# gengshan-y/ppr-diffphys

Hardware: AMD Instinct MI355X
Metric: env-steps/sec (fwd+adjoint), Laikago 12-DoF, batch=4096, 1/2/4/8 MI355X (higher is better)
Workload: dtype f32; 1 GPU; laikago, mixed mi-trot/mi-spin mocap targets, 4096 envs in total (4096 on rank 0) x 100 sim steps (4 frames), dt=5e-4, fwd+adjoint, batch split only (no collective); global_batch=4096, envs_per_gpu=4096, sim_steps=100, segment_lanes=16, nan_grads=0

## Files before the change

### ppr-diffphys_amd/csrc/pd_args.h

```cpp
#pragma once
#include "pd_device.h"
#include "pd_trajloss.h"

#define PD_BWAVES 4
#define PD_BLOCK (2 * PD_BWAVES * 64)
#define PD_FK_BLOCK (PD_BWAVES * 64)
#define PD_BLOCK3 (3 * PD_BWAVES * 64)

#define PD_HITLOG 32

enum { PD_K_ROLLOUT_FWD = 0, PD_K_ROLLOUT_BWD = 1, PD_K_FK_FWD = 2, PD_K_FK_BWD = 3,
       PD_K_REDUCE_FK = 4, PD_K_SEEDS_FK = 5 };
#define PD_REDUCE_BLOCK 1024

constexpr bool pd_split(int jt) { return jt == PD_JT_REVOLUTE; }
constexpr bool pd_parented(int jt) { return jt == PD_JT_REVOLUTE || jt == PD_JT_COMPOUND; }
enum { PD_KV_FWD_SPLIT = 0, PD_KV_FWD_UNSPLIT, PD_KV_BWD_2ROLE, PD_KV_BWD3_2ROLE, PD_KV_FK,
       PD_KV_FWD_QUAD, PD_KV_BWD_QUAD };
struct PdLaunchCfg {
  int kernel;
  int roles;
  int groups;
  int nblocks, threads;
  size_t lds;
};
inline int pd_groups_per_wg(int n_groups, int cu_count) {
  int g = cu_count > 0 ? (n_groups + cu_count - 1) / cu_count : PD_BWAVES;
  return g < 1 ? 1 : (g > PD_BWAVES ? PD_BWAVES : g);
}
inline int pd_kernel_variant(int kind, int jt, int n_groups, int cu_count) {
  if (kind == PD_K_ROLLOUT_FWD) return (jt != PD_JT_COMPOUND || n_groups <= PD_BWAVES * cu_count) ? PD_KV_FWD_SPLIT : PD_KV_FWD_UNSPLIT;
  if (kind == PD_K_ROLLOUT_BWD) {
    return pd_split(jt) ? PD_KV_BWD_2ROLE : PD_KV_BWD3_2ROLE;
  }
  return PD_KV_FK;
}
#define PD_CULLW_MIN_CAP 48
inline int pd_fwd_cull_cap(int nb, int segw, int list_cap, int env_lds_floats, int rec, int w6) {
  const int spec_off = ((4 + rec + 2 * w6) * nb + w6 + 3) & ~3;
  return env_lds_floats - (spec_off + 8 * nb + 4 + list_cap + 8 * segw + 6 * segw + 8 * segw);
}
inline int pd_variant_roles(int kv) {
  return (kv == PD_KV_FWD_UNSPLIT || kv == PD_KV_FK) ? 1 : 2;
}

#define PD_TRAJ_FLOATS 20

struct RolloutArgs {
  int bs, nsteps, nframes;
  float dt;
  const float *q_init, *qd_init, *torques, *res_f, *refs, *target_ke, *target_kd, *inv_mass, *inertia, *inv_inertia;
  const float *state0;
  float *g_state0;
  const int *frame_of_step;
  float *ws;
  float *wp_pos, *wp_vel, *grf, *jaf;
  const float *adj_pos, *adj_vel;
  float *g_q_init, *g_qd_init, *g_torques, *g_res_f, *g_refs, *g_ke, *g_kd, *g_inv_mass, *g_inertia, *g_inv_inertia;
  int *hitlog;
  const float *loss_target;
  const unsigned char *loss_outseq;
  float loss_rot_ratio;
  float *loss_seed_pos, *loss_seed_gt, *loss_table;
  unsigned long long *dbg;
};


struct FkArgs {
  int n;
  const float *joint_q, *joint_qd;
  float *body_q, *body_qd;
  const float *adj_body_q, *adj_body_qd;
  float *g_joint_q, *g_joint_qd;
  int perm_bs;
};
struct ReduceFkArgs { FkArgs fk; TrajReduceArgs red; int in_lds; };
struct SeedsFkArgs { FkArgs fk; TrajSeedsArgs seeds; };

// ... 14 lines not shown
```

### ppr-diffphys_amd/csrc/pd_host.hip

```cpp
#include <algorithm>
#include <cmath>
#include <cstdio>
#include <cstring>
#include <string>
#include <vector>

#include "../../include/ppr_diffphys.h"
#include "pd_args.h"

static thread_local std::string g_err;
static int fail(const std::string &msg) { g_err = msg; return 1; }
__attribute__((visibility("hidden"))) int pd_set_error(const char *msg) { return fail(msg); }
static int hip_fail(hipError_t e, const char *what) { return fail(std::string(what) + ": " + hipGetErrorString(e)); }

struct pd_model {
  int nb = 0, nq = 0, nqd = 0, nc = 0, nmat = 0;
  std::vector<int> jtype, jparent, qstart, qdstart, cbody, cmat;
  std::vector<float> X_p, X_c, axis, com, lim_lo, lim_hi, lim_ke, lim_kd, cpoint, cdist, materials;
  float gravity[3] = {0, 0, 0}, attach_ke = 0, attach_kd = 0;
  int segw = 0, jt = 0;
  std::vector<int> contact_order;
  struct Quad { void *blob; PdDevModel dev; size_t lds_tables; int jt; };
  Quad *quad = nullptr;
  int policy = 0;
// ... 270 lines not shown
  void *blob = nullptr;
  hipError_t e = hipMalloc(&blob, b.buf.size());
  if (e != hipSuccess) return hip_fail(e, "hipMalloc(model)");
  e = hipMemcpy(blob, b.buf.data(), b.buf.size(), hipMemcpyHostToDevice);
  if (e != hipSuccess) { (void)hipFree(blob); return hip_fail(e, "hipMemcpy(model)"); }
  b.point(d, (const unsigned char *)blob);
  free_device(m);
  m->blob = blob; m->dev = d;
  m->lds_tables = lds_tables; m->lds_max = (size_t)lds_max;
  m->segw = segw; m->jt = ch.jt; m->contact_order = t.order;
  return 0;
}

static void build_quad(pd_model *m) {
  free_quad(m);
  if (m->jt != PD_JT_REVOLUTE || m->nb > 16) return;
  pd_model tmp = *m;
  tmp.blob = nullptr; tmp.quad = nullptr;
  if (build_device(&tmp, 64, m->dev.global_tables != 0) != 0 || tmp.jt != PD_JT_REVOLUTE) { if (tmp.blob) (void)hipFree(tmp.blob); return; }
  m->quad = new pd_model::Quad{tmp.blob, tmp.dev, tmp.lds_tables, tmp.jt};
}

static int g_groups = 0;

static bool use_quad(const pd_model *m, int kind, int n_envs) {
  if (!m->quad || m->family == 1 || (kind != PD_K_ROLLOUT_FWD && kind != PD_K_ROLLOUT_BWD)) return false;
  return m->family == 2 || n_envs <= (kind == PD_K_ROLLOUT_FWD ? PD_BWAVES : PD_BWAVES / 2) * m->quad->dev.cu_count;
}

struct LaunchPlan { PdLaunchCfg cfg; const PdDevModel *dev; int jt, policy, wi, info[4]; };
static void finish_cfg(PdLaunchCfg &c, const PdDevModel &d, int n_groups, int epw, size_t tab, int lead, size_t lead_lds) {
  c.nblocks = lead + (n_groups + c.groups - 1) / c.groups;
  c.threads = c.roles * c.groups * 64;
  c.lds = std::max(lead_lds, variant_lds(d, c.kernel, (size_t)c.groups * epw, tab));
}
static LaunchPlan plan_launch(const pd_model *m, int kind, int n_envs, bool loss) {
  const bool rollout = kind <= PD_K_ROLLOUT_BWD, fwd = kind == PD_K_ROLLOUT_FWD, quad = use_quad(m, kind, n_envs);
  const PdDevModel &d = quad ? m->quad->dev : m->dev;
  const int segw = quad ? 64 : m->segw, jt = quad ? m->quad->jt : m->jt;
  const int epw = 64 / segw, n_groups = (n_envs + epw - 1) / epw;
  bool cullw = pd_fwd_cull_cap(d.nb, segw, d.list_cap, d.env_lds_floats, PD_REC, PD_W6) >= PD_CULLW_MIN_CAP;
#ifdef PD_NO_CULLW
  cullw = false;
#endif
  PdLaunchCfg c{};
  if (quad) {
    c.kernel = fwd ? PD_KV_FWD_QUAD : PD_KV_BWD_QUAD;
    c.roles = fwd && !cullw ? 2 : 3;
  } else {
    c.kernel = pd_kernel_variant(kind, jt, n_groups, d.cu_count);
    if (loss && c.kernel == PD_KV_FWD_UNSPLIT) c.kernel = PD_KV_FWD_SPLIT;
    if (d.global_tables && c.kernel == PD_KV_FWD_UNSPLIT) c.kernel = PD_KV_FWD_SPLIT;
    c.roles = c.kernel == PD_KV_FWD_SPLIT && jt == PD_JT_REVOLUTE && cullw ? 3 : pd_variant_roles(c.kernel);
  }
  c.groups = !rollout ? PD_BWAVES : (g_groups ? g_groups : pd_groups_per_wg(n_groups, d.cu_count));
  if (c.kernel == PD_KV_BWD_QUAD && c.groups > 2) c.groups = 2;
  finish_cfg(c, d, n_groups, epw, d.global_tables ? 0 : (quad ? m->quad->lds_tables : m->lds_tables), 0, 0);
  return LaunchPlan{c, &d, jt, rollout && m->policy == PD_NUM_LITERAL ? 1 : 0, width_index(segw), {c.nblocks, c.threads, (int)c.lds, c.groups * epw}};
}

static hipError_t launch(const pd_model *m, int kind, const void *args, int n_envs, hipStream_t st) {
  const LaunchPlan p = plan_launch(m, kind, n_envs, kind == PD_K_ROLLOUT_FWD && ((const RolloutArgs *)args)->loss_target != nullptr);
  if (p.cfg.nblocks == 0) return hipSuccess;
  if (kind <= PD_K_ROLLOUT_BWD) std::copy(p.info, p.info + 4, const_cast<pd_model *>(m)->last_launch[kind]);
  return g_launch[p.policy][p.wi](kind, p.jt, *p.dev, args, p.cfg, st);
}

static void timing_begin(pd_model *m, int kind, hipStream_t st) {
  if (!m->timing) return;
  if (!m->ev[kind][0]) { (void)hipEventCreate(&m->ev[kind][0]); (void)hipEventCreate(&m->ev[kind][1]); }
  (void)hipEventRecord(m->ev[kind][0], st);
}
static void timing_end(pd_model *m, int kind, hipStream_t st) {
  if (!m->timing) return;
  (void)hipEventRecord(m->ev[kind][1], st);
  m->ev_valid[kind] = true;
}

static int frame_table(pd_model *m, int nsteps, int nframes, const int *f2s, const int **out, hipStream_t st) {
  if (nframes < 0) return fail("negative frame count");
  if (nframes > 0 && !f2s) return fail("null frame2step");
  std::vector<int> fos((size_t)nsteps + 1, -1);
  for (int f = 0; f < nframes; ++f) {
    const int s = f2s[f];
    if (s < 0 || s > nsteps)
      return fail("frame2step[" + std::to_string(f) + "] = " + std::to_string(s) + " is outside 0.." + std::to_string(nsteps));
    if (fos[s] >= 0)
      return fail("frame2step names step " + std::to_string(s) + " twice (frames " + std::to_string(fos[s]) + " and " + std::to_string(f) + ")");
    fos[s] = f;
  }
  for (const auto &e : m->fos)
    if (e.nsteps == nsteps && (int)e.f2s.size() == nframes && std::equal(e.f2s.begin(), e.f2s.end(), f2s)) { *out = e.dev; return 0; }
  if (m->fos.size() >= 4096) return fail("more than 4096 distinct (nsteps, frame2step) tables on one model; destroy and recreate the model");
  {
    hipStreamCaptureStatus cs = hipStreamCaptureStatusNone;
    if (st != nullptr && hipStreamIsCapturing(st, &cs) == hipSuccess && cs != hipStreamCaptureStatusNone)
      return fail("a new (nsteps, frame2step) needs a synchronous upload, which a stream capture in progress forbids: warm up first");
  }
  int *dev = nullptr;
  hipError_t e = hipMalloc((void **)&dev, fos.size() * sizeof(int));
  if (e != hipSuccess) return hip_fail(e, "hipMalloc(frame table)");
  e = hipMemcpy(dev, fos.data(), fos.size() * sizeof(int), hipMemcpyHostToDevice);
  if (e != hipSuccess) { (void)hipFree(dev); return hip_fail(e, "hipMemcpy(frame table)"); }
  m->fos.push_back({nsteps, std::vector<int>(f2s, f2s + nframes), dev});
  *out = dev;
  return 0;
// ... 377 lines not shown
```

### ppr-diffphys_amd/csrc/pd_kernels.hip

```cpp
#include "pd_device.h"
#include "pd_args.h"
#include "pd_se3.h"
#include "pd_quad.h"

#if PD_POLICY == 1
#define k_rollout_fwd k_rollout_fwd_literal
#define k_rollout_bwd k_rollout_bwd_literal
#define k_rollout_bwd3 k_rollout_bwd3_literal
#define PD_LAUNCH_NAME(w) PD_CAT(PD_CAT(pd_launch_seg, w), _literal)
#define PD_SET_LDS_NAME(w) PD_CAT(PD_CAT(pd_set_lds_seg, w), _literal)
#else
#define PD_LAUNCH_NAME(w) PD_CAT(pd_launch_seg, w)
#define PD_SET_LDS_NAME(w) PD_CAT(pd_set_lds_seg, w)
#endif

#ifdef PD_STAMPS
#define STAMP_DECL unsigned long long st_acc[16] = {0, 0, 0, 0, 0, 0, 0, 0, 0, 0, 0, 0, 0, 0, 0, 0}, st_t = pd_memtime()
#define STAMP_ARGS , unsigned long long *st_acc, unsigned long long &st_t
#define STAMP_PASS , st_acc, st_t
#define STAMP(i) do { unsigned long long t2_ = pd_memtime(); st_acc[i] += t2_ - st_t; st_t = t2_; } while (0)
#define STAMP_COUNT(i, n) do { st_acc[i] += (unsigned long long)(n); } while (0)
#define STAMP_FLUSH(a) do { if ((a).dbg && (threadIdx.x & 63) == 0) for (int i_ = 0; i_ < 16; ++i_) (a).dbg[((size_t)blockIdx.x * (blockDim.x / 64) + (threadIdx.x >> 6)) * 16 + i_] = st_acc[i_]; } while (0)
__device__ __forceinline__ unsigned long long pd_memtime() {
  unsigned long long t;
  __builtin_amdgcn_sched_barrier(0);
  asm volatile("s_memtime %0\n\ts_waitcnt lgkmcnt(0)" : "=s"(t)::"memory");
  __builtin_amdgcn_sched_barrier(0);
  return t;
}
#else
#define STAMP_DECL
#define STAMP(i)
#define STAMP_COUNT(i, n)
#define STAMP_FLUSH(a)
#define STAMP_ARGS
#define STAMP_PASS
#endif


#define PD_WAIT_VMEM() __builtin_amdgcn_s_waitcnt(0x0F70)

typedef const __attribute__((address_space(4))) int *pd_const_int_p;
#define PD_OPAQUE_V(x) asm volatile("" : "+v"(x))
#define PD_OPAQUE_S(x) do { if constexpr (CLONE && SEGW < 64) asm volatile("" : "+s"(x)); } while (0)
PD_DEV int ld_uniform(const int *p, int i) { return ((pd_const_int_p)(unsigned long long)p)[i]; }
PD_DEV float ldg(const float *ubase, unsigned boff) { return *(const float *)((const char *)ubase + boff); }
PD_DEV void stg(float *ubase, unsigned boff, float v) { *(float *)((char *)ubase + boff) = v; }
PD_DEV float4 ldg4(const float *ubase, unsigned boff) { return *(const float4 *)((const char *)ubase + boff); }
PD_DEV void stg4(float *ubase, unsigned boff, float4 v) { *(float4 *)((char *)ubase + boff) = v; }
PD_DEV float2 ldg2(const float *ubase, unsigned boff) { return *(const float2 *)((const char *)ubase + boff); }
PD_DEV void stg2(float *ubase, unsigned boff, float2 v) { *(float2 *)((char *)ubase + boff) = v; }
template <bool ON>
PD_DEV bool ptr_given(const float *p) {
  if constexpr (ON) return p != nullptr;
  else return true;
}

#define PD_TRAJ_G 5

#define NZ(x) grad_post<1>(x)

PD_DEV void add_frame_seeds(const RolloutArgs &a, int fr, int N, size_t idx, BodyAdj &gn) {
  const float *gp = a.adj_pos + ((size_t)fr * N + idx) * 7, *gv = a.adj_vel + ((size_t)fr * N + idx) * 6;
  gn.p += V3(gp[0], gp[1], gp[2]); gn.r += Q4(gp[3], gp[4], gp[5], gp[6]);
  gn.w += V3(gv[0], gv[1], gv[2]); gn.v += V3(gv[3], gv[4], gv[5]);
}

template <int SEGW>
struct Seg {
  static constexpr int EPW = 64 / SEGW;
  static constexpr unsigned long long MASK = SEGW == 64 ? ~0ull : ((1ull << SEGW) - 1ull);
};

struct SegMask { unsigned lo, hi; };
template <int SEGW>
PD_DEV SegMask seg_mask(int seg) {
  unsigned long long mk = Seg<SEGW>::MASK << (seg * SEGW);
  SegMask s; s.lo = (unsigned)mk; s.hi = (unsigned)(mk >> 32);
  return s;
}
PD_DEV int seg_slot(bool pred, SegMask sm, int &total) {
  unsigned long long b = __ballot(pred);
  unsigned lo = (unsigned)b & sm.lo, hi = (unsigned)(b >> 32) & sm.hi;
  int slot = total + (int)__builtin_amdgcn_mbcnt_hi(hi, __builtin_amdgcn_mbcnt_lo(lo, 0u));
  total += __popc(lo) + __popc(hi);
  return slot;
}

template <int NV>
PD_DEV void seg_run_sum(float *acc, int pb, int l, int nh, bool &last) {
  const int pbp = __builtin_amdgcn_update_dpp(-1, pb, 0x138, 0xf, 0xf, false);
  const int pbn = __builtin_amdgcn_update_dpp(-1, pb, 0x130, 0xf, 0xf, false);
  const bool in = l < nh, start = in && (l == 0 || pbp != pb);
  last = in && (l == nh - 1 || pbn != pb);
  const int lane = (int)(threadIdx.x & 63);
  const unsigned long long starts = __ballot(start), below = starts & ((2ull << lane) - 1ull);
  const int pos = in ? lane - (63 - __clzll((long long)below)) : -1;
  float x[NV];
#pragma unroll
  for (int i = 0; i < NV; ++i) x[i] = acc[i];
  for (int it = 1; __ballot(pos >= it) != 0ull; ++it) {
    const bool upd = pos >= it;
#pragma unroll
    for (int i = 0; i < NV; ++i) {
// ... 1109 lines not shown
    if (wr) {
      float4 cv = stage_record(rec, cull, b, s, rc, Rm);
      if (SPLIT && (step + 1) % PD_SPEC_K == 0) {
        margin = sink_margin<JT, SPEC_STEPS>(m, c, s, a.dt);
        if (CULLW) { sunk_n = 0.f; margin98_n = c.sphere.w >= 0.0f ? 0.98f * margin : __builtin_inff(); }
        else { sunk = 0.f; margin98 = c.sphere.w >= 0.0f ? 0.98f * margin : __builtin_inff(); }
        cv.x -= margin;
        spec[(((step + 1) / PD_SPEC_K) & 1) * nb + b] = cv;
      }
    }
    if (!SPLIT) WAVE_SYNC();
    STAMP(5);
  }
  if (a.nsteps > 0) spill_wrench(a.nsteps - 1);
  {
    const int fr_last = ld_uniform(a.frame_of_step, a.nsteps);
    if (fr_last >= 0 && is_body) {
      float *o = a.wp_pos + ((size_t)fr_last * N + idx) * 7;
      o[0] = s.p.x; o[1] = s.p.y; o[2] = s.p.z; o[3] = s.r.x; o[4] = s.r.y; o[5] = s.r.z; o[6] = s.r.w;
      o = a.wp_vel + ((size_t)fr_last * N + idx) * 6;
      o[0] = s.w.x; o[1] = s.w.y; o[2] = s.w.z; o[3] = s.v.x; o[4] = s.v.y; o[5] = s.v.z;
#pragma unroll
      for (int k = 0; k < 6; ++k) {
        if (a.grf) a.grf[((size_t)fr_last * N + idx) * 6 + k] = 0.f;
        if (a.jaf) a.jaf[((size_t)fr_last * N + idx) * 6 + k] = 0.f;
      }
    }
  }
  if constexpr (LOSS) {
    for (int f = 0; f < a.nframes; ++f) {
      BodyState cs = s;
      if (is_body) {
        const float *o = a.wp_pos + ((size_t)f * N + idx) * 7;
        cs.p = V3(o[0], o[1], o[2]); cs.r = Q4(o[3], o[4], o[5], o[6]);
      }
      frame_loss(f, cs);
    }
  }
  STAMP_FLUSH(a);
}

#ifdef PD_KNOCK
#undef pair_wait
#if !(PD_KNOCK & 16)
#define pair_wait(f, v) pair_wait_knock(f, v, knock_role)
#endif
#endif
template <bool SEL>
__device__ __forceinline__ bool grad_wanted(const float *g) {
  if constexpr (SEL) return g != nullptr;
  else return true;
}

template <int SEGW, int JT, bool QUAD = false, bool SEL = false>
__global__ __launch_bounds__(PD_BLOCK) void k_rollout_bwd(PdDevModel m, RolloutArgs a) {
  static_assert(JT == PD_JT_REVOLUTE, "the wave-specialised adjoint of revolute-only plain models: every jointed body is a revolute joint on a parent body");
  extern __shared__ __attribute__((aligned(16))) unsigned char smem[];
  constexpr int EPW = Seg<SEGW>::EPW;
  const int bw = (int)blockDim.x / (QUAD ? 192 : 128);
  const int role = (int)(threadIdx.x >> 6) / bw;
  const bool contact_wave = role != 0;
  [[maybe_unused]] const int knock_role = role;
  const int lane = threadIdx.x & 63, wave = (int)(threadIdx.x >> 6) % bw;
  const int seg = lane / SEGW, l = lane % SEGW;
  const int env = (blockIdx.x * bw + wave) * EPW + seg;
  const bool env_ok = env < a.bs;
  const int ec = env_ok ? env : 0;
  const bool is_body = env_ok && l < m.nb;
  const int b = l < m.nb ? l : m.nb - 1;
  const int nb = m.nb, N = a.bs * nb;

  SweepTables tabs;
  const int env_stride = m.env_lds_floats + 2 * m.env_lds_jc + (QUAD ? m.env_lds_rec2 : 0);
  float *scratch = lds_setup<false>(m, smem, tabs, wave * EPW + seg, env_stride);
  float4 *cull = (float4 *)scratch;
  float *rec = scratch + 4 * nb, *adjf = rec + nb * PD_REC, *cslot = adjf + nb * PD_W6, *cacc = cslot + (nb + 1) * PD_ADJ;
  int *list = (int *)(cacc + nb * PD_ADJ), *hits = list + m.list_cap;
  float *slot = (float *)(hits + PD_HIT_CAP_TILES * SEGW);
  float *jc = scratch + m.env_lds_floats;
  int *sig = (int *)(scratch - (size_t)seg * env_stride + m.env_lds_floats - 4);
  if (lane == 0 && !contact_wave) { sig[0] = 0; sig[1] = 0; sig[2] = 0; sig[3] = 0; }
  __syncthreads();
  PD_KNOCK_EXIT(false, knock_role);
  if constexpr (QUAD) {
    if (!env_ok) return;
  }

  BodyConst c = load_body_const(m, b, ec);
#pragma unroll
  for (int u = 0; u < 4; ++u) c.small_e[u] = m.small_tiles[u * 64 + (l < 64 ? l : 0)];
  if (l == 0) {
#pragma unroll
    for (int k = 0; k < PD_ADJ; ++k) cslot[nb * PD_ADJ + k] = 0.f;
  }
  int cz[4];
#pragma unroll
  for (int k = 0; k < 4; ++k) cz[k] = is_body && c.child[k] >= 0 ? c.child[k] : nb;
  const float *rec_s = rec;
  const float4 *cull_s = cull;
  auto contact_hit = [&](const float *r, float4 P, float4 mat, float *out) {
    const int pb = (int)(r - rec_s) / PD_REC;
    BodyAdj o = adj_zero();
    if constexpr (QUAD) {
      ContactPre C = contact_point_adj_pre(r, cull_s[pb], P, mat);
      contact_pre_barrier(C);
      contact_point_adj_rest(C, P, mat, ld3(adjf + pb * PD_W6), ld3(adjf + pb * PD_W6 + 3), o);
    } else {
      contact_point_adj(r, cull_s[pb], P, mat, ld3(adjf + pb * PD_W6), ld3(adjf + pb * PD_W6 + 3), o);
    }
    adj_store(out, o);
  };
  if (contact_wave) {
    STAMP_DECL;
    const bool rev = is_body && c.type == PD_JOINT_REVOLUTE;
    const size_t qd_off = (size_t)ec * m.nqd + c.qdstart;
    const float ke1 = rev ? a.target_ke[qd_off] : 0.f, kd1 = rev ? a.target_kd[qd_off] : 0.f;
    const int lq = l < PD_HITLOG - 1 ? l : PD_HITLOG - 2;
    const unsigned boff_c = (unsigned)((size_t)ec * nb + b) * 4u, boff_p = (unsigned)((size_t)ec * nb + (c.parent >= 0 ? c.parent : b)) * 4u;
    const unsigned boff_qd = (unsigned)qd_off * 4u, boff_lg = (unsigned)ec * (PD_HITLOG * 4u);
    auto load_log = [&](int step, int &cnt, int &e) {
// ... 395 lines not shown
            if (cid != 0xff) adj_add_from(gs, cslot + cid * PD_ADJ);
          }
          BodyAdj pr_ = fk_joint_adj<JT, 1>(c, a.q_init + (size_t)ec * m.nq + c.qstart, a.qd_init + (size_t)ec * m.nqd + c.qdstart, rec0,
                                          gs, a.g_q_init + (size_t)ec * m.nq + c.qstart, a.g_qd_init + (size_t)ec * m.nqd + c.qdstart);
          adj_store(cslot + b * PD_ADJ, pr_);
        }
        WAVE_SYNC();
      }
    }
    if (qbody) {
      if (qc == 0) a.g_inv_mass[qidx] = NZ(g_inv_m);
      if (k.isv) {
        float *gi = a.g_inertia + qidx * 9 + qc * 3, *gj = a.g_inv_inertia + qidx * 9 + qc * 3;
        gi[0] = NZ(g_I.a); gi[1] = NZ(g_I.b); gi[2] = NZ(g_I.c);
        gj[0] = NZ(g_invI.a); gj[1] = NZ(g_invI.b); gj[2] = NZ(g_invI.c);
      }
      const size_t og = (size_t)ec * m.nqd + B.qdstart;
      if (B.type == PD_JOINT_REVOLUTE && qc == 0) { a.g_ke[og] = NZ(g_ke); a.g_kd[og] = NZ(g_kd); }
      if (B.type == PD_JOINT_FREE) {
        a.g_ke[og + qc] = 0.f; a.g_kd[og + qc] = 0.f;
        if (qc < 2) { a.g_ke[og + 4 + qc] = 0.f; a.g_kd[og + 4 + qc] = 0.f; }
      }
    }
    return;
  }
  constexpr int ND = 1;
  const size_t idx = (size_t)ec * nb + b;
  const int ndof = c.type == PD_JOINT_REVOLUTE ? 1 : (c.type == PD_JOINT_COMPOUND ? 3 : 0);

  float inv_m = a.inv_mass[idx], I[9], invI[9], ke[ND], kd[ND];
#pragma unroll
  for (int k = 0; k < 9; ++k) { I[k] = a.inertia[idx * 9 + k]; invI[k] = a.inv_inertia[idx * 9 + k]; }
#pragma unroll
  for (int k = 0; k < ND; ++k) {
    bool on = k < ndof;
    ke[k] = on ? a.target_ke[(size_t)ec * m.nqd + c.qdstart + k] : 0.f;
    kd[k] = on ? a.target_kd[(size_t)ec * m.nqd + c.qdstart + k] : 0.f;
  }
  float g_inv_m = 0.f, g_I[9], g_invI[9], g_ke[ND], g_kd[ND];
#pragma unroll
  for (int k = 0; k < 9; ++k) { g_I[k] = 0.f; g_invI[k] = 0.f; }
#pragma unroll
  for (int k = 0; k < ND; ++k) { g_ke[k] = 0.f; g_kd[k] = 0.f; }
  if (is_body) {
#pragma unroll
    for (int k = 0; k < PD_ADJ; ++k) cacc[b * PD_ADJ + k] = 0.f;
  }

  BodyAdj gn = adj_zero();
  BodyState s;
  s.p = V3(0, 0, 0); s.r = Q4(0, 0, 0, 1); s.w = V3(0, 0, 0); s.v = V3(0, 0, 0);

  const unsigned boff = (unsigned)idx * 4u, boff_qd = (unsigned)((size_t)ec * m.nqd + c.qdstart) * 4u;
  const bool zero_by_lanes = m.jtype[0] == PD_JOINT_FREE && nb >= 7;
  const unsigned boff_zero = (unsigned)((size_t)ec * m.nqd + m.qdstart[0] + (b >= 1 && b <= 6 ? b - 1 : 0)) * 4u;
  float4 n_s[PD_TRAJ_G];
  float n_tgt[ND];
  int n_fr = -1;
  auto load_step = [&](int step) {
    const int sc = __builtin_amdgcn_readfirstlane(step >= 0 ? step : 0);
    n_fr = a.frame_of_step[sc + 1];
    const float *tj = a.ws + (size_t)sc * (PD_TRAJ_G * 4) * N;
#pragma unroll
    for (int g = 0; g < PD_TRAJ_G; ++g) n_s[g] = ldg4(tj + (size_t)(4 * g) * N, boff * 4u);
    const size_t o = (size_t)sc * a.bs * m.nqd;
#pragma unroll
    for (int k = 0; k < ND; ++k) {
      bool on = k < ndof;
      n_tgt[k] = on ? ldg(a.refs + o + k, boff_qd) : 0.f;
    }
  };
  if (a.nsteps > 0) load_step(a.nsteps - 1);
  STAMP_DECL;
  for (int step = a.nsteps - 1; step >= 0; --step) {
    PD_WAIT_VMEM();
    {
      const int fr = n_fr;
      if (fr >= 0) {
        add_frame_seeds(a, fr, N, idx, gn);
      }
    }
    s.r = Q4(n_s[0].x, n_s[0].y, n_s[0].z, n_s[0].w); s.w = V3(n_s[1].x, n_s[1].y, n_s[1].z);
    s.p = V3(n_s[2].x, n_s[2].y, n_s[2].z); s.v = V3(n_s[1].w, n_s[2].w, n_s[3].x);
    v3 t0 = V3(n_s[3].y, n_s[3].z, n_s[3].w), f0 = V3(n_s[4].x, n_s[4].y, n_s[4].z);
    const unsigned clamp_mask = __float_as_uint(n_s[4].w);
    float tgt[ND];
#pragma unroll
    for (int k = 0; k < ND; ++k) tgt[k] = n_tgt[k];
    const size_t oc = (size_t)step * a.bs * m.nqd;
    load_step(step - 1);
    float Rm[9];
    rotm(s.r, Rm);
    const v3 rc = mat_vec(Rm, c.com);
    if (is_body) stage_record(rec, cull, b, s, rc, Rm);
    STAMP(0);
    BodyAdj ga = adj_zero();
    v3 adj_t0 = V3(0, 0, 0), adj_f0 = adj_t0;
    float aR[9];
#pragma unroll
    for (int k = 0; k < 9; ++k) aR[k] = 0.f;
    integrate_adj(m, c, s, Rm, clamp_mask, t0, f0, inv_m, I, invI, a.dt, gn, ga, aR, adj_t0, adj_f0, g_inv_m, g_I, g_invI);
    if (is_body) {
      float *f = adjf + b * PD_W6;
      f[0] = adj_t0.x; f[1] = adj_t0.y; f[2] = adj_t0.z; f[3] = adj_f0.x; f[4] = adj_f0.y; f[5] = adj_f0.z;
    }
    STAMP(1);
    pair_signal(sig, a.nsteps - step);
    if (grad_wanted<SEL>(a.g_res_f) && is_body) {
      float *o = a.g_res_f + (size_t)step * N * 6;
      stg2(o, boff * 6u, make_float2(NZ(adj_t0.x), NZ(adj_t0.y))); stg2(o + 2, boff * 6u, make_float2(NZ(adj_t0.z), NZ(adj_f0.x)));
      stg2(o + 4, boff * 6u, make_float2(NZ(adj_f0.y), NZ(adj_f0.z)));
    }
    pair_wait(sig + 1, a.nsteps - step);
    BodyAdj par = adj_zero();
    float a_tgt[ND], a_act[ND], a_ke[ND], a_kd[ND];
#pragma unroll
    for (int k = 0; k < ND; ++k) { a_tgt[k] = 0.f; a_act[k] = 0.f; a_ke[k] = 0.f; a_kd[k] = 0.f; }
    if (is_body && c.type != PD_JOINT_FREE) {
      const v3 gp_t = ld3(adjf + c.parent * PD_W6), gp_f = ld3(adjf + c.parent * PD_W6 + 3);
      const RevCache R = rev_cache_load(jc + (step & 1) * m.env_lds_jc + b * PD_JC);
      rev_adjoint<true>(m, c, s, rc, rec, R, tgt[0], ke[0], kd[0], adj_t0, adj_f0, gp_t, gp_f, ga, par, aR, a_tgt[0], a_act[0], a_ke[0], a_kd[0]);
    }
    rotm_adj(s.r, aR, ga.r);
    if (is_body) {
      adj_store(cslot + b * PD_ADJ, par);
#pragma unroll
      for (int k = 0; k < ND; ++k) {
        if (k < ndof) {
          if (grad_wanted<SEL>(a.g_refs)) stg(a.g_refs + oc + k, boff_qd, NZ(a_tgt[k]));
          if (grad_wanted<SEL>(a.g_torques)) stg(a.g_torques + oc + k, boff_qd, NZ(a_act[k]));
        }
        g_ke[k] += a_ke[k]; g_kd[k] += a_kd[k];
      }
      if (zero_by_lanes) {
        if (b >= 1 && b <= 6) {
          if (grad_wanted<SEL>(a.g_refs)) stg(a.g_refs + oc, boff_zero, 0.f);
          if (grad_wanted<SEL>(a.g_torques)) stg(a.g_torques + oc, boff_zero, 0.f);
        }
      } else if (c.type == PD_JOINT_FREE) {
#pragma unroll
        for (int k = 0; k < 6; ++k) {
          if (grad_wanted<SEL>(a.g_refs)) stg(a.g_refs + oc + k, boff_qd, 0.f);
          if (grad_wanted<SEL>(a.g_torques)) stg(a.g_torques + oc + k, boff_qd, 0.f);
        }
      }
    }
    STAMP(2);
    WAVE_SYNC();
    {
      const float *const src[4] = {cslot + cz[0] * PD_ADJ, cslot + cz[1] * PD_ADJ, cslot + cz[2] * PD_ADJ, cslot + cz[3] * PD_ADJ};
      adj_add_from_n(ga, src);
    }
    for (int k = 4; k < m.max_children; ++k) {
      int cid = (int)((c.children >> (8 * k)) & 0xffull);
      if (is_body && cid != 0xff) adj_add_from(ga, cslot + cid * PD_ADJ);
    }
    STAMP(3);
    pair_wait(sig + 2, a.nsteps - step);
    if (is_body) {
      float *d = cacc + b * PD_ADJ;
      const float *const src[1] = {d};
      adj_add_from_n(ga, src);
#pragma unroll
      for (int k = 0; k < PD_ADJ; ++k) d[k] = 0.f;
    }
    gn = ga;
    STAMP(4);
  }
  STAMP_FLUSH(a);
  {
    int fr = a.frame_of_step[0];
    if (fr >= 0) {
      add_frame_seeds(a, fr, N, idx, gn);
    }
  }
  if (a.g_state0 && is_body) adj_store(a.g_state0 + idx * PD_ADJ, gn);
  const int fk_levels = a.g_state0 ? -1 : m.max_depth;
  if (a.nsteps == 0) {
    for (int d = 0; d <= fk_levels; ++d) {
      if (is_body && c.depth == d) {
        s = fk_joint<JT>(c, a.q_init + (size_t)ec * m.nq + c.qstart, a.qd_init + (size_t)ec * m.nqd + c.qdstart, rec);
        stage_record(rec, b, s, c.com);
      }
      WAVE_SYNC();
    }
  }
  for (int d = fk_levels; d >= 0; --d) {
    if (is_body && c.depth == d) {
      for (int k = 0; k < m.max_children; ++k) {
        int cid = (int)((c.children >> (8 * k)) & 0xffull);
        if (cid != 0xff) adj_add_from(gn, cslot + cid * PD_ADJ);
      }
      BodyAdj par = fk_joint_adj<JT, 1>(c, a.q_init + (size_t)ec * m.nq + c.qstart, a.qd_init + (size_t)ec * m.nqd + c.qdstart, rec,
                                     gn, a.g_q_init + (size_t)ec * m.nq + c.qstart, a.g_qd_init + (size_t)ec * m.nqd + c.qdstart);
      adj_store(cslot + b * PD_ADJ, par);
    }
    WAVE_SYNC();
  }
  if (is_body) {
    a.g_inv_mass[idx] = NZ(g_inv_m);
#pragma unroll
    for (int k = 0; k < 9; ++k) { a.g_inertia[idx * 9 + k] = NZ(g_I[k]); a.g_inv_inertia[idx * 9 + k] = NZ(g_invI[k]); }
    const size_t og = (size_t)ec * m.nqd + c.qdstart;
#pragma unroll
    for (int k = 0; k < ND; ++k)
      if (k < ndof) { a.g_ke[og + k] = NZ(g_ke[k]); a.g_kd[og + k] = NZ(g_kd[k]); }
    if (c.type == PD_JOINT_FREE) {
#pragma unroll
      for (int k = 0; k < 6; ++k) { a.g_ke[og + k] = 0.f; a.g_kd[og + k] = 0.f; }
    }
  }
}

template <int SEGW, int JT, bool GT = false, bool SEL = false>
__global__ __launch_bounds__(PD_BLOCK) void k_rollout_bwd3(PdDevModel m, RolloutArgs a) {
  extern __shared__ __attribute__((aligned(16))) unsigned char smem[];
  constexpr int EPW = Seg<SEGW>::EPW;
  constexpr int ND = (JT & PD_JT_COMPOUND) ? 3 : 1;
  static_assert(JT != PD_JT_REVOLUTE, "revolute-only models take k_rollout_bwd");
  const int bw = (int)blockDim.x / (64 * 2);
  const int lane = threadIdx.x & 63, wave_id = threadIdx.x >> 6;
  const int role = wave_id / bw ? 2 : 0, wave = wave_id % bw;
  [[maybe_unused]] const int knock_role = role;
  const int seg = lane / SEGW, l = lane % SEGW;
  const int env = (blockIdx.x * bw + wave) * EPW + seg;
  const bool env_ok = env < a.bs;
  const int ec = env_ok ? env : 0;
  const bool is_body = env_ok && l < m.nb;
  const int b = l < m.nb ? l : m.nb - 1;
  const int nb = m.nb, N = a.bs * nb;

  SweepTables tabs;
  float *scratch = lds_setup<!GT>(m, smem, tabs, wave * EPW + seg, m.env_lds_bwd3);
  float4 *const cull0 = (float4 *)scratch;
  float *const rec0 = scratch + 8 * nb;
  float4 *cull = cull0;
  float *rec = rec0;
  auto select_step = [&](int step) { rec = rec0 + (step & 1) * nb * PD_REC; cull = cull0 + (step & 1) * nb; };
  float *adjf = rec0 + 2 * nb * PD_REC, *cslot = adjf + nb * PD_W6, *oslot = cslot + (nb + 1) * PD_ADJ;
  float *cacc = oslot + nb * PD_ADJ;
  float *gacc = cacc + nb * PD_ADJ;
  int *list = (int *)(gacc + (nb + 1) * PD_GACC), *hits = list + m.list_cap;
  float *slot = (float *)(hits + PD_HIT_CAP_TILES * SEGW);
  int *sig = (int *)(scratch - (size_t)seg * m.env_lds_bwd3 + m.env_lds_bwd3 - 4);
  if (role == 0) {
    if (lane == 0) { sig[0] = 0; sig[1] = 0; sig[2] = 0; sig[3] = 0; }
    if (is_body) {
#pragma unroll
      for (int k = 0; k < PD_ADJ; ++k) { cacc[b * PD_ADJ + k] = 0.f; oslot[b * PD_ADJ + k] = 0.f; cslot[b * PD_ADJ + k] = 0.f; }
    }
    if (l == 0) {
#pragma unroll
      for (int k = 0; k < PD_ADJ; ++k) cslot[nb * PD_ADJ + k] = 0.f;
    }
  }
  __syncthreads();
  PD_KNOCK_EXIT(false, knock_role);

  const size_t idx = (size_t)ec * nb + b;
  const unsigned boff = (unsigned)idx * 4u;
// ... 345 lines not shown
template <int SEGW, int JT>
__global__ __launch_bounds__(PD_REDUCE_BLOCK) void k_reduce_fk(PdDevModel m, ReduceFkArgs a) {
  extern __shared__ __attribute__((aligned(16))) unsigned char smem[];
  if (blockIdx.x == 0) {
    if (a.in_lds) traj_loss_reduce_block<true>(a.red, (float *)smem);
    else traj_loss_reduce_block<false>(a.red, (float *)smem);
    return;
  }
  fk_chain<SEGW, JT, false>(m, a.fk, smem, blockIdx.x - 1);
}
template <int SEGW, int JT>
__global__ __launch_bounds__(PD_FK_BLOCK) void k_seeds_fk(PdDevModel m, SeedsFkArgs a) {
  extern __shared__ __attribute__((aligned(16))) unsigned char smem[];
  if ((int)blockIdx.x < a.seeds.nblocks) { traj_seeds_block(a.seeds, blockIdx.x); return; }
  fk_chain<SEGW, JT, true>(m, a.fk, smem, blockIdx.x - a.seeds.nblocks);
}

#ifndef PD_SEGW
#error "compile with -DPD_SEGW=16, 32 or 64"
#endif
#define PD_CAT2(a, b) a##b
#define PD_CAT(a, b) PD_CAT2(a, b)


typedef void (*RolloutKernel)(PdDevModel, RolloutArgs);
static const int kFwdVariants[] = {PD_KV_FWD_SPLIT, PD_KV_FWD_UNSPLIT, PD_KV_FWD_QUAD}, kBwdVariants[] = {PD_KV_BWD_2ROLE, PD_KV_BWD3_2ROLE, PD_KV_BWD_QUAD};

template <int JT, bool GT, bool SAVE, bool ZC>
static RolloutKernel select_fwd(int kernel, int roles, bool runsum, bool loss) {
  if (kernel == PD_KV_FWD_QUAD) {
    if constexpr (PD_SEGW == 64 && JT == PD_JT_REVOLUTE) {
      if (roles == 3) return loss ? k_rollout_fwd<PD_SEGW, JT, true, true, true, true, false, GT, SAVE, ZC> : k_rollout_fwd<PD_SEGW, JT, true, false, true, true, false, GT, SAVE, ZC>;
      return loss ? k_rollout_fwd<PD_SEGW, JT, true, true, true, false, false, GT, SAVE, ZC> : k_rollout_fwd<PD_SEGW, JT, true, false, true, false, false, GT, SAVE, ZC>;
    } else {
      return nullptr;
    }
  }
  if (roles == 3) {
    if constexpr (JT == PD_JT_REVOLUTE) {
      if (runsum) return loss ? k_rollout_fwd<PD_SEGW, JT, true, true, false, true, true, GT, SAVE, ZC> : k_rollout_fwd<PD_SEGW, JT, true, false, false, true, true, GT, SAVE, ZC>;
      return loss ? k_rollout_fwd<PD_SEGW, JT, true, true, false, true, false, GT, SAVE, ZC> : k_rollout_fwd<PD_SEGW, JT, true, false, false, true, false, GT, SAVE, ZC>;
    } else {
      return nullptr;
    }
  }
  if (loss)
    return kernel == PD_KV_FWD_SPLIT ? k_rollout_fwd<PD_SEGW, JT, true, true, false, false, false, GT, SAVE, ZC> : nullptr;
  if (kernel == PD_KV_FWD_SPLIT || JT != PD_JT_COMPOUND) return k_rollout_fwd<PD_SEGW, JT, true, false, false, false, false, GT, SAVE, ZC>;
  if constexpr (JT == PD_JT_COMPOUND && !GT) return k_rollout_fwd<PD_SEGW, JT, false, false, false, false, false, false, SAVE, ZC>;
  else return nullptr;
}

template <int JT, bool GT, bool SEL>
static RolloutKernel select_bwd(int kernel) {
  if constexpr (pd_split(JT)) {
    if (kernel == PD_KV_BWD_QUAD) {
      if constexpr (PD_SEGW == 64) return k_rollout_bwd<PD_SEGW, JT, true, SEL>;
      else return nullptr;
    }
    return k_rollout_bwd<PD_SEGW, JT, false, SEL>;
  } else {
    return k_rollout_bwd3<PD_SEGW, JT, GT, SEL>;
  }
}

static hipError_t launch_rollout(RolloutKernel k, const PdDevModel &m, const RolloutArgs &a, const PdLaunchCfg &cfg, hipStream_t st) {
  if (!k) return hipErrorInvalidValue;
  hipLaunchKernelGGL(k, dim3(cfg.nblocks), dim3(cfg.threads), cfg.lds, st, m, a);
  return hipGetLastError();
}
template <int JT, bool GT, bool SAVE, bool ZC>
static hipError_t launch_fwd(const PdDevModel &m, const RolloutArgs &a, const PdLaunchCfg &cfg, hipStream_t st) {
  return launch_rollout(select_fwd<JT, GT, SAVE, ZC>(cfg.kernel, cfg.roles, cfg.groups >= PD_BWAVES, a.loss_target != nullptr), m, a, cfg, st);
}
template <int JT, bool GT, bool SEL>
static hipError_t launch_bwd(const PdDevModel &m, const RolloutArgs &a, const PdLaunchCfg &cfg, hipStream_t st) {
  return launch_rollout(select_bwd<JT, GT, SEL>(cfg.kernel), m, a, cfg, st);
}

template <int JT, bool GT>
static hipError_t launch_jt(int kind, const PdDevModel &m, const void *args, const PdLaunchCfg &cfg, hipStream_t st) {
  [[maybe_unused]] const dim3 g(cfg.nblocks), t(cfg.threads);
  [[maybe_unused]] const size_t lds = cfg.lds;
  switch (kind) {
    case PD_K_ROLLOUT_FWD: {
      const RolloutArgs &a = *(const RolloutArgs *)args;
      if (a.nsteps > 0 && (!a.torques || !a.res_f))
        return a.ws ? launch_fwd<JT, GT, true, true>(m, a, cfg, st) : launch_fwd<JT, GT, false, true>(m, a, cfg, st);
      return a.ws || a.nsteps == 0 ? launch_fwd<JT, GT, true, false>(m, a, cfg, st) : launch_fwd<JT, GT, false, false>(m, a, cfg, st);
    }
    case PD_K_ROLLOUT_BWD: {
      const RolloutArgs &a = *(const RolloutArgs *)args;
      return a.nsteps > 0 && (!a.g_torques || !a.g_res_f || !a.g_refs || !a.torques) ? launch_bwd<JT, GT, true>(m, a, cfg, st) : launch_bwd<JT, GT, false>(m, a, cfg, st);
    }
#if PD_POLICY == 0
    case PD_K_FK_FWD:
      hipLaunchKernelGGL((k_fk<PD_SEGW, JT, false>), g, t, lds, st, m, *(const FkArgs *)args);
      break;
    case PD_K_FK_BWD:
      hipLaunchKernelGGL((k_fk<PD_SEGW, JT, true>), g, t, lds, st, m, *(const FkArgs *)args);
      break;
    case PD_K_REDUCE_FK:
      hipLaunchKernelGGL((k_reduce_fk<PD_SEGW, JT>), g, t, lds, st, m, *(const ReduceFkArgs *)args);
      break;
    case PD_K_SEEDS_FK:
      hipLaunchKernelGGL((k_seeds_fk<PD_SEGW, JT>), g, t, lds, st, m, *(const SeedsFkArgs *)args);
      break;
#endif
    default:
      return hipErrorInvalidValue;
  }
  return hipGetLastError();
}

static hipError_t set_lds(RolloutKernel k, int bytes) {
  return k ? hipFuncSetAttribute((const void *)k, hipFuncAttributeMaxDynamicSharedMemorySize, bytes) : hipSuccess;
}
template <int JT, bool GT, bool SAVE, bool ZC>
static hipError_t set_lds_fwd(int bytes) {
  for (const int kernel : kFwdVariants)
    for (int roles = 1; roles <= 3; ++roles)
      for (int flags = 0; flags < 4; ++flags)
        if (const hipError_t e = set_lds(select_fwd<JT, GT, SAVE, ZC>(kernel, roles, (flags & 1) != 0, (flags & 2) != 0), bytes)) return e;
  return hipSuccess;
}
template <int JT, bool GT, bool SEL>
static hipError_t set_lds_bwd(int bytes) {
  for (const int kernel : kBwdVariants)
    if (const hipError_t e = set_lds(select_bwd<JT, GT, SEL>(kernel), bytes)) return e;
  return hipSuccess;
}

template <int JT, bool GT>
static hipError_t set_lds_gt(int bytes) {
  hipError_t e;
  if ((e = set_lds_fwd<JT, GT, true, false>(bytes))) return e;
  if ((e = set_lds_fwd<JT, GT, false, false>(bytes))) return e;
  if ((e = set_lds_fwd<JT, GT, true, true>(bytes))) return e;
  if ((e = set_lds_fwd<JT, GT, false, true>(bytes))) return e;
  if ((e = set_lds_bwd<JT, GT, false>(bytes))) return e;
  if ((e = set_lds_bwd<JT, GT, true>(bytes))) return e;
#if PD_POLICY == 0
  if constexpr (GT) return hipSuccess;
  if ((e = hipFuncSetAttribute((const void *)k_fk<PD_SEGW, JT, false>, hipFuncAttributeMaxDynamicSharedMemorySize, bytes))) return e;
  if ((e = hipFuncSetAttribute((const void *)k_reduce_fk<PD_SEGW, JT>, hipFuncAttributeMaxDynamicSharedMemorySize, bytes))) return e;
  if ((e = hipFuncSetAttribute((const void *)k_seeds_fk<PD_SEGW, JT>, hipFuncAttributeMaxDynamicSharedMemorySize, bytes))) return e;
  return hipFuncSetAttribute((const void *)k_fk<PD_SEGW, JT, true>, hipFuncAttributeMaxDynamicSharedMemorySize, bytes);
#else
  return hipSuccess;
#endif
}

template <int JT>
static hipError_t set_lds_jt(int bytes) {
  const hipError_t e = set_lds_gt<JT, false>(bytes);
  return e != hipSuccess ? e : set_lds_gt<JT, true>(bytes);
}

hipError_t PD_LAUNCH_NAME(PD_SEGW)(int kind, int jt, const PdDevModel &m, const void *args, const PdLaunchCfg &cfg, hipStream_t st) {
  if (m.global_tables) {
    if (jt == PD_JT_REVOLUTE) return launch_jt<PD_JT_REVOLUTE, true>(kind, m, args, cfg, st);
    if (jt == PD_JT_COMPOUND) return launch_jt<PD_JT_COMPOUND, true>(kind, m, args, cfg, st);
    return launch_jt<PD_JT_REVOLUTE | PD_JT_COMPOUND | PD_JT_FIXED, true>(kind, m, args, cfg, st);
  }
  if (jt == PD_JT_REVOLUTE) return launch_jt<PD_JT_REVOLUTE, false>(kind, m, args, cfg, st);
  if (jt == PD_JT_COMPOUND) return launch_jt<PD_JT_COMPOUND, false>(kind, m, args, cfg, st);
  return launch_jt<PD_JT_REVOLUTE | PD_JT_COMPOUND | PD_JT_FIXED, false>(kind, m, args, cfg, st);
}
hipError_t PD_SET_LDS_NAME(PD_SEGW)(int jt, int bytes) {
  if (jt == PD_JT_REVOLUTE) return set_lds_jt<PD_JT_REVOLUTE>(bytes);
  if (jt == PD_JT_COMPOUND) return set_lds_jt<PD_JT_COMPOUND>(bytes);
  return set_lds_jt<PD_JT_REVOLUTE | PD_JT_COMPOUND | PD_JT_FIXED>(bytes);
}
```

Baseline: 906.8 million env-steps/s.

## Add TREE4 specialised adjoint rollout kernel for free-root trees with at most four children

Adds a TREE4 template variant of the backward rollout kernel, chosen on the host when the model's root is a free joint, every body has at most four children and there are at least seven bodies. The variant drops the extra-children loop and the free-joint zeroing branch, keeps per-step output row pointers in scalar registers via an address-space cast with an inline-asm constraint, and restructures the step prefetch into a lambda with a StepIn struct. After the loop it recomputes lane and body constants instead of keeping them live across the loop, which is meant to lower vector register pressure. The cost is one more kernel instantiation per configuration and reliance on the compiler honouring the scalar-pointer hint.

Result: no change. 908.8 million env-steps/s, median of 5 (+0.2%).

```diff
diff --git a/ppr-diffphys_amd/csrc/pd_args.h b/ppr-diffphys_amd/csrc/pd_args.h
--- a/ppr-diffphys_amd/csrc/pd_args.h
+++ b/ppr-diffphys_amd/csrc/pd_args.h
@@ -23,7 +23,9 @@
   int groups;
   int nblocks, threads;
   size_t lds;
+  int tree4;
 };
+inline bool pd_tree4(int max_children, int root_type, int nb) { return max_children <= 4 && root_type == PD_JOINT_FREE && nb >= 7; }
 inline int pd_groups_per_wg(int n_groups, int cu_count) {
   int g = cu_count > 0 ? (n_groups + cu_count - 1) / cu_count : PD_BWAVES;
   return g < 1 ? 1 : (g > PD_BWAVES ? PD_BWAVES : g);
diff --git a/ppr-diffphys_amd/csrc/pd_host.hip b/ppr-diffphys_amd/csrc/pd_host.hip
--- a/ppr-diffphys_amd/csrc/pd_host.hip
+++ b/ppr-diffphys_amd/csrc/pd_host.hip
@@ -346,6 +346,7 @@
     if (loss && c.kernel == PD_KV_FWD_UNSPLIT) c.kernel = PD_KV_FWD_SPLIT;
     if (d.global_tables && c.kernel == PD_KV_FWD_UNSPLIT) c.kernel = PD_KV_FWD_SPLIT;
     c.roles = c.kernel == PD_KV_FWD_SPLIT && jt == PD_JT_REVOLUTE && cullw ? 3 : pd_variant_roles(c.kernel);
+    c.tree4 = c.kernel == PD_KV_BWD_2ROLE && pd_tree4(d.max_children, m->jtype[0], d.nb);
   }
   c.groups = !rollout ? PD_BWAVES : (g_groups ? g_groups : pd_groups_per_wg(n_groups, d.cu_count));
   if (c.kernel == PD_KV_BWD_QUAD && c.groups > 2) c.groups = 2;
diff --git a/ppr-diffphys_amd/csrc/pd_kernels.hip b/ppr-diffphys_amd/csrc/pd_kernels.hip
--- a/ppr-diffphys_amd/csrc/pd_kernels.hip
+++ b/ppr-diffphys_amd/csrc/pd_kernels.hip
@@ -50,6 +50,16 @@
 PD_DEV void stg4(float *ubase, unsigned boff, float4 v) { *(float4 *)((char *)ubase + boff) = v; }
 PD_DEV float2 ldg2(const float *ubase, unsigned boff) { return *(const float2 *)((const char *)ubase + boff); }
 PD_DEV void stg2(float *ubase, unsigned boff, float2 v) { *(float2 *)((char *)ubase + boff) = v; }
+typedef __attribute__((address_space(1))) float gfloat;
+typedef __attribute__((address_space(1))) char gchar;
+PD_DEV gfloat *scalar_ptr(float *p) {
+  gfloat *g = (gfloat *)p;
+  asm("" : "+s"(g));
+  return g;
+}
+PD_DEV void stg(gfloat *ubase, unsigned boff, float v) { *(gfloat *)((gchar *)ubase + boff) = v; }
+typedef float pd_f2v __attribute__((ext_vector_type(2)));
+PD_DEV void stg2(gfloat *ubase, unsigned boff, float2 v) { *(__attribute__((address_space(1))) pd_f2v *)((gchar *)ubase + boff) = pd_f2v{v.x, v.y}; }
 template <bool ON>
 PD_DEV bool ptr_given(const float *p) {
   if constexpr (ON) return p != nullptr;
@@ -1265,8 +1275,9 @@
   else return true;
 }
 
-template <int SEGW, int JT, bool QUAD = false, bool SEL = false>
+template <int SEGW, int JT, bool QUAD = false, bool SEL = false, bool TREE4 = false>
 __global__ __launch_bounds__(PD_BLOCK) void k_rollout_bwd(PdDevModel m, RolloutArgs a) {
+  static_assert(!(QUAD && TREE4), "TREE4 is a flag of the lane-per-body body wave");
   static_assert(JT == PD_JT_REVOLUTE, "the wave-specialised adjoint of revolute-only plain models: every jointed body is a revolute joint on a parent body");
   extern __shared__ __attribute__((aligned(16))) unsigned char smem[];
   constexpr int EPW = Seg<SEGW>::EPW;
@@ -1279,6 +1290,7 @@
   const int env = (blockIdx.x * bw + wave) * EPW + seg;
   const bool env_ok = env < a.bs;
   const int ec = env_ok ? env : 0;
+  [[maybe_unused]] const int env_w = __builtin_amdgcn_readfirstlane(env - seg);
   const bool is_body = env_ok && l < m.nb;
   const int b = l < m.nb ? l : m.nb - 1;
   const int nb = m.nb, N = a.bs * nb;
@@ -1780,43 +1792,51 @@
   s.p = V3(0, 0, 0); s.r = Q4(0, 0, 0, 1); s.w = V3(0, 0, 0); s.v = V3(0, 0, 0);
 
   const unsigned boff = (unsigned)idx * 4u, boff_qd = (unsigned)((size_t)ec * m.nqd + c.qdstart) * 4u;
-  const bool zero_by_lanes = m.jtype[0] == PD_JOINT_FREE && nb >= 7;
+  const bool zero_by_lanes = TREE4 || (m.jtype[0] == PD_JOINT_FREE && nb >= 7);
   const unsigned boff_zero = (unsigned)((size_t)ec * m.nqd + m.qdstart[0] + (b >= 1 && b <= 6 ? b - 1 : 0)) * 4u;
-  float4 n_s[PD_TRAJ_G];
-  float n_tgt[ND];
-  int n_fr = -1;
-  auto load_step = [&](int step) {
+  struct StepIn {
+    float4 s[PD_TRAJ_G];
+    float tgt[ND];
+    int fr;
+  };
+  StepIn in;
+  in.fr = -1;
+  auto load_step = [&](int step, StepIn &n) {
     const int sc = __builtin_amdgcn_readfirstlane(step >= 0 ? step : 0);
-    n_fr = a.frame_of_step[sc + 1];
+    n.fr = a.frame_of_step[sc + 1];
     const float *tj = a.ws + (size_t)sc * (PD_TRAJ_G * 4) * N;
 #pragma unroll
-    for (int g = 0; g < PD_TRAJ_G; ++g) n_s[g] = ldg4(tj + (size_t)(4 * g) * N, boff * 4u);
+    for (int g = 0; g < PD_TRAJ_G; ++g) n.s[g] = ldg4(tj + (size_t)(4 * g) * N, boff * 4u);
     const size_t o = (size_t)sc * a.bs * m.nqd;
 #pragma unroll
     for (int k = 0; k < ND; ++k) {
       bool on = k < ndof;
-      n_tgt[k] = on ? ldg(a.refs + o + k, boff_qd) : 0.f;
+      n.tgt[k] = on ? ldg(a.refs + o + k, boff_qd) : 0.f;
     }
   };
-  if (a.nsteps > 0) load_step(a.nsteps - 1);
   STAMP_DECL;
-  for (int step = a.nsteps - 1; step >= 0; --step) {
+  auto body_step = [&](const int step, const StepIn &cur, StepIn &nxt) __attribute__((always_inline)) {
     PD_WAIT_VMEM();
     {
-      const int fr = n_fr;
+      const int fr = cur.fr;
       if (fr >= 0) {
         add_frame_seeds(a, fr, N, idx, gn);
       }
     }
-    s.r = Q4(n_s[0].x, n_s[0].y, n_s[0].z, n_s[0].w); s.w = V3(n_s[1].x, n_s[1].y, n_s[1].z);
-    s.p = V3(n_s[2].x, n_s[2].y, n_s[2].z); s.v = V3(n_s[1].w, n_s[2].w, n_s[3].x);
-    v3 t0 = V3(n_s[3].y, n_s[3].z, n_s[3].w), f0 = V3(n_s[4].x, n_s[4].y, n_s[4].z);
-    const unsigned clamp_mask = __float_as_uint(n_s[4].w);
+    s.r = Q4(cur.s[0].x, cur.s[0].y, cur.s[0].z, cur.s[0].w); s.w = V3(cur.s[1].x, cur.s[1].y, cur.s[1].z);
+    s.p = V3(cur.s[2].x, cur.s[2].y, cur.s[2].z); s.v = V3(cur.s[1].w, cur.s[2].w, cur.s[3].x);
+    v3 t0 = V3(cur.s[3].y, cur.s[3].z, cur.s[3].w), f0 = V3(cur.s[4].x, cur.s[4].y, cur.s[4].z);
+    const unsigned clamp_mask = __float_as_uint(cur.s[4].w);
     float tgt[ND];
 #pragma unroll
-    for (int k = 0; k < ND; ++k) tgt[k] = n_tgt[k];
+    for (int k = 0; k < ND; ++k) tgt[k] = cur.tgt[k];
     const size_t oc = (size_t)step * a.bs * m.nqd;
-    load_step(step - 1);
+    auto row_ptr = [](float *p) {
+      if constexpr (TREE4) return scalar_ptr(p);
+      else return p;
+    };
+    const auto o_refs = row_ptr(a.g_refs + oc), o_torques = row_ptr(a.g_torques + oc);
+    load_step(step - 1, nxt);
     float Rm[9];
     rotm(s.r, Rm);
     const v3 rc = mat_vec(Rm, c.com);
@@ -1835,7 +1855,7 @@
     STAMP(1);
     pair_signal(sig, a.nsteps - step);
     if (grad_wanted<SEL>(a.g_res_f) && is_body) {
-      float *o = a.g_res_f + (size_t)step * N * 6;
+      const auto o = row_ptr(a.g_res_f + (size_t)step * N * 6);
       stg2(o, boff * 6u, make_float2(NZ(adj_t0.x), NZ(adj_t0.y))); stg2(o + 2, boff * 6u, make_float2(NZ(adj_t0.z), NZ(adj_f0.x)));
       stg2(o + 4, boff * 6u, make_float2(NZ(adj_f0.y), NZ(adj_f0.z)));
     }
@@ -1855,21 +1875,21 @@
 #pragma unroll
       for (int k = 0; k < ND; ++k) {
         if (k < ndof) {
-          if (grad_wanted<SEL>(a.g_refs)) stg(a.g_refs + oc + k, boff_qd, NZ(a_tgt[k]));
-          if (grad_wanted<SEL>(a.g_torques)) stg(a.g_torques + oc + k, boff_qd, NZ(a_act[k]));
+          if (grad_wanted<SEL>(a.g_refs)) stg(o_refs + k, boff_qd, NZ(a_tgt[k]));
+          if (grad_wanted<SEL>(a.g_torques)) stg(o_torques + k, boff_qd, NZ(a_act[k]));
         }
         g_ke[k] += a_ke[k]; g_kd[k] += a_kd[k];
       }
       if (zero_by_lanes) {
         if (b >= 1 && b <= 6) {
-          if (grad_wanted<SEL>(a.g_refs)) stg(a.g_refs + oc, boff_zero, 0.f);
-          if (grad_wanted<SEL>(a.g_torques)) stg(a.g_torques + oc, boff_zero, 0.f);
-        }
-      } else if (c.type == PD_JOINT_FREE) {
+          if (grad_wanted<SEL>(a.g_refs)) stg(o_refs, boff_zero, 0.f);
+          if (grad_wanted<SEL>(a.g_torques)) stg(o_torques, boff_zero, 0.f);
+        }
+      } else if (!TREE4 && c.type == PD_JOINT_FREE) {
 #pragma unroll
         for (int k = 0; k < 6; ++k) {
-          if (grad_wanted<SEL>(a.g_refs)) stg(a.g_refs + oc + k, boff_qd, 0.f);
-          if (grad_wanted<SEL>(a.g_torques)) stg(a.g_torques + oc + k, boff_qd, 0.f);
+          if (grad_wanted<SEL>(a.g_refs)) stg(o_refs + k, boff_qd, 0.f);
+          if (grad_wanted<SEL>(a.g_torques)) stg(o_torques + k, boff_qd, 0.f);
         }
       }
     }
@@ -1879,9 +1899,11 @@
       const float *const src[4] = {cslot + cz[0] * PD_ADJ, cslot + cz[1] * PD_ADJ, cslot + cz[2] * PD_ADJ, cslot + cz[3] * PD_ADJ};
       adj_add_from_n(ga, src);
     }
-    for (int k = 4; k < m.max_children; ++k) {
-      int cid = (int)((c.children >> (8 * k)) & 0xffull);
-      if (is_body && cid != 0xff) adj_add_from(ga, cslot + cid * PD_ADJ);
+    if constexpr (!TREE4) {
+      for (int k = 4; k < m.max_children; ++k) {
+        int cid = (int)((c.children >> (8 * k)) & 0xffull);
+        if (is_body && cid != 0xff) adj_add_from(ga, cslot + cid * PD_ADJ);
+      }
     }
     STAMP(3);
     pair_wait(sig + 2, a.nsteps - step);
@@ -1894,46 +1916,54 @@
     }
     gn = ga;
     STAMP(4);
-  }
+  };
+  if (a.nsteps > 0) load_step(a.nsteps - 1, in);
+  for (int step = a.nsteps - 1; step >= 0; --step) body_step(step, in, in);
   STAMP_FLUSH(a);
+  const int lane_ = (int)__builtin_amdgcn_mbcnt_hi(~0u, __builtin_amdgcn_mbcnt_lo(~0u, 0u));
+  const int env_ = env_w + lane_ / SEGW, l_ = lane_ % SEGW;
+  const int ec_ = env_ < a.bs ? env_ : 0, b_ = l_ < nb ? l_ : nb - 1;
+  const BodyConst cb = load_body_const(m, b_, ec_);
+  const size_t idx_ = (size_t)ec_ * nb + b_;
+  const int ndof_ = cb.type == PD_JOINT_REVOLUTE ? 1 : (cb.type == PD_JOINT_COMPOUND ? 3 : 0);
   {
     int fr = a.frame_of_step[0];
     if (fr >= 0) {
-      add_frame_seeds(a, fr, N, idx, gn);
-    }
-  }
-  if (a.g_state0 && is_body) adj_store(a.g_state0 + idx * PD_ADJ, gn);
+      add_frame_seeds(a, fr, N, idx_, gn);
+    }
+  }
+  if (a.g_state0 && is_body) adj_store(a.g_state0 + idx_ * PD_ADJ, gn);
   const int fk_levels = a.g_state0 ? -1 : m.max_depth;
   if (a.nsteps == 0) {
     for (int d = 0; d <= fk_levels; ++d) {
-      if (is_body && c.depth == d) {
-        s = fk_joint<JT>(c, a.q_init + (size_t)ec * m.nq + c.qstart, a.qd_init + (size_t)ec * m.nqd + c.qdstart, rec);
-        stage_record(rec, b, s, c.com);
+      if (is_body && cb.depth == d) {
+        s = fk_joint<JT>(cb, a.q_init + (size_t)ec_ * m.nq + cb.qstart, a.qd_init + (size_t)ec_ * m.nqd + cb.qdstart, rec);
+        stage_record(rec, b_, s, cb.com);
       }
       WAVE_SYNC();
     }
   }
   for (int d = fk_levels; d >= 0; --d) {
-    if (is_body && c.depth == d) {
+    if (is_body && cb.depth == d) {
       for (int k = 0; k < m.max_children; ++k) {
-        int cid = (int)((c.children >> (8 * k)) & 0xffull);
+        int cid = (int)((cb.children >> (8 * k)) & 0xffull);
         if (cid != 0xff) adj_add_from(gn, cslot + cid * PD_ADJ);
       }
-      BodyAdj par = fk_joint_adj<JT, 1>(c, a.q_init + (size_t)ec * m.nq + c.qstart, a.qd_init + (size_t)ec * m.nqd + c.qdstart, rec,
-                                     gn, a.g_q_init + (size_t)ec * m.nq + c.qstart, a.g_qd_init + (size_t)ec * m.nqd + c.qdstart);
-      adj_store(cslot + b * PD_ADJ, par);
+      BodyAdj par = fk_joint_adj<JT, 1>(cb, a.q_init + (size_t)ec_ * m.nq + cb.qstart, a.qd_init + (size_t)ec_ * m.nqd + cb.qdstart, rec,
+                                     gn, a.g_q_init + (size_t)ec_ * m.nq + cb.qstart, a.g_qd_init + (size_t)ec_ * m.nqd + cb.qdstart);
+      adj_store(cslot + b_ * PD_ADJ, par);
     }
     WAVE_SYNC();
   }
   if (is_body) {
-    a.g_inv_mass[idx] = NZ(g_inv_m);
-#pragma unroll
-    for (int k = 0; k < 9; ++k) { a.g_inertia[idx * 9 + k] = NZ(g_I[k]); a.g_inv_inertia[idx * 9 + k] = NZ(g_invI[k]); }
-    const size_t og = (size_t)ec * m.nqd + c.qdstart;
+    a.g_inv_mass[idx_] = NZ(g_inv_m);
+#pragma unroll
+    for (int k = 0; k < 9; ++k) { a.g_inertia[idx_ * 9 + k] = NZ(g_I[k]); a.g_inv_inertia[idx_ * 9 + k] = NZ(g_invI[k]); }
+    const size_t og = (size_t)ec_ * m.nqd + cb.qdstart;
 #pragma unroll
     for (int k = 0; k < ND; ++k)
-      if (k < ndof) { a.g_ke[og + k] = NZ(g_ke[k]); a.g_kd[og + k] = NZ(g_kd[k]); }
-    if (c.type == PD_JOINT_FREE) {
+      if (k < ndof_) { a.g_ke[og + k] = NZ(g_ke[k]); a.g_kd[og + k] = NZ(g_kd[k]); }
+    if (cb.type == PD_JOINT_FREE) {
 #pragma unroll
       for (int k = 0; k < 6; ++k) { a.g_ke[og + k] = 0.f; a.g_kd[og + k] = 0.f; }
     }
@@ -2385,13 +2415,13 @@
 }
 
 template <int JT, bool GT, bool SEL>
-static RolloutKernel select_bwd(int kernel) {
+static RolloutKernel select_bwd(int kernel, bool tree4) {
   if constexpr (pd_split(JT)) {
     if (kernel == PD_KV_BWD_QUAD) {
       if constexpr (PD_SEGW == 64) return k_rollout_bwd<PD_SEGW, JT, true, SEL>;
       else return nullptr;
     }
-    return k_rollout_bwd<PD_SEGW, JT, false, SEL>;
+    return tree4 ? k_rollout_bwd<PD_SEGW, JT, false, SEL, true> : k_rollout_bwd<PD_SEGW, JT, false, SEL, false>;
   } else {
     return k_rollout_bwd3<PD_SEGW, JT, GT, SEL>;
   }
@@ -2408,7 +2438,7 @@
 }
 template <int JT, bool GT, bool SEL>
 static hipError_t launch_bwd(const PdDevModel &m, const RolloutArgs &a, const PdLaunchCfg &cfg, hipStream_t st) {
-  return launch_rollout(select_bwd<JT, GT, SEL>(cfg.kernel), m, a, cfg, st);
+  return launch_rollout(select_bwd<JT, GT, SEL>(cfg.kernel, cfg.tree4 != 0), m, a, cfg, st);
 }
 
 template <int JT, bool GT>
@@ -2460,7 +2490,8 @@
 template <int JT, bool GT, bool SEL>
 static hipError_t set_lds_bwd(int bytes) {
   for (const int kernel : kBwdVariants)
-    if (const hipError_t e = set_lds(select_bwd<JT, GT, SEL>(kernel), bytes)) return e;
+    for (int tree4 = 0; tree4 < 2; ++tree4)
+      if (const hipError_t e = set_lds(select_bwd<JT, GT, SEL>(kernel, tree4 != 0), bytes)) return e;
   return hipSuccess;
 }
 
```
